# rust-bio/rust-bio

Measured on NVIDIA H100. Metric: GCUPS, higher is better.
Workload: dtype int32

## Files before the change

rust_bio_b200/csrc/b2a_common.cuh:

```cuda
#pragma once
#include <stdint.h>

#if defined(__CUDACC__)
#define B2A_HD __host__ __device__ __forceinline__
#else
#define B2A_HD inline
struct int4 { int x, y, z, w; };
struct int2 { int x, y; };
struct uint4 { unsigned x, y, z, w; };
inline int4 make_int4(int x, int y, int z, int w) { return int4{x, y, z, w}; }
inline int2 make_int2(int x, int y) { return int2{x, y}; }
#endif

namespace b2a {

#if defined(B2A_HOST_WARP) && !defined(__CUDACC__)
struct HostWarp {
  long long x[32];
  void (*next_lane)(void*);
  void* harness;
  void (*other_warp)(void*);
};
inline HostWarp* host_warp = nullptr;
inline int host_lane = 0;
// ... 51 lines not shown
  uint32_t uniform;
  uint32_t nstrips;
  uint32_t xwords;
  uint32_t ywords;
  uint32_t K;
  uint32_t rows_pad;
  uint64_t seq_off;
  uint64_t bnd_off;
  uint64_t rows_off;
  uint64_t rowm_off;
  uint64_t tb_off;
  uint64_t ops_off;
  uint64_t strip_task_base;
};

enum { ROWS_SN = 0, ROWS_LY = 1, ROWS_SL = 2, ROWS_IL = 3, ROWS_NL = 4, ROWS_ARRAYS = 5 };

B2A_HD int32_t imax(int32_t a, int32_t b) { return a > b ? a : b; }


B2A_HD int32_t col0_I(const DevScoring& sc, int32_t i) {
  if (i == 1) return sc.gap_open;
  return imax(sc.gap_open + sc.gap_extend * (i - 1), sc.xclip_prefix + sc.gap_open);
}
B2A_HD uint32_t col0_ibits(const DevScoring& sc, int32_t i) {
  if (i == 1) return TB_START;
  return (sc.gap_open + sc.gap_extend * (i - 1) > sc.xclip_prefix + sc.gap_open) ? TB_INS
                                                                                   : TB_XCLIP_PREFIX;
}
B2A_HD int32_t col0_S(const DevScoring& sc, int32_t i) {
  return imax(col0_I(sc, i), sc.xclip_prefix);
}
B2A_HD uint32_t col0_sbits(const DevScoring& sc, int32_t i) {
  return sc.xclip_prefix > col0_I(sc, i) ? TB_XCLIP_PREFIX : TB_INS;
}
B2A_HD int32_t row0_D(const DevScoring& sc, int32_t j) {
  if (j == 1) return sc.gap_open;
  return imax(sc.gap_open + sc.gap_extend * (j - 1), sc.yclip_prefix + sc.gap_open);
}
B2A_HD uint32_t row0_dbits(const DevScoring& sc, int32_t j) {
  if (j == 1) return TB_START;
  return (sc.gap_open + sc.gap_extend * (j - 1) > sc.yclip_prefix + sc.gap_open) ? TB_DEL
                                                                                   : TB_YCLIP_PREFIX;
}
B2A_HD int32_t row0_S(const DevScoring& sc, int32_t j, int32_t n) {
  int32_t s = imax(row0_D(sc, j), sc.yclip_prefix);
  if (j == n && sc.yclip_suffix > s) s = sc.yclip_suffix;
  return s;
}
B2A_HD uint32_t row0_sbits(const DevScoring& sc, int32_t j, int32_t n) {
  if (j == 0) return TB_START;
  const int32_t d = row0_D(sc, j);
  uint32_t b = d > sc.yclip_prefix ? TB_DEL : TB_YCLIP_PREFIX;
  if (j == n && sc.yclip_suffix > imax(d, sc.yclip_prefix)) b = TB_YCLIP_SUFFIX;
  return b;
}
B2A_HD int32_t xclip_score(const DevScoring& sc, int32_t j) {
  return sc.xclip_prefix + imax(sc.yclip_prefix, sc.gap_open + sc.gap_extend * (j - 1));
}

B2A_HD int64_t bnd_index(int32_t G, int32_t j, int32_t pi, int32_t maxn) {
  return G < 32 ? (int64_t)j * 32 + pi : (int64_t)pi * (maxn + 1) + j;
}

B2A_HD int32_t pack_s16x2(int32_t lo, int32_t hi) {
#if defined(__CUDA_ARCH__)
  return (int32_t)__byte_perm((uint32_t)lo, (uint32_t)hi, 0x5410);
#else
  return (int32_t)(((uint32_t)hi << 16) | ((uint32_t)lo & 0xffffu));
#endif
}
B2A_HD int32_t lo_s16(int32_t w) { return (int32_t)(int16_t)(uint16_t)((uint32_t)w & 0xffffu); }
B2A_HD int32_t hi_s16(int32_t w) { return w >> 16; }

#if defined(__CUDACC__)
__host__ __device__
#endif
constexpr int lut_entries(int alpha) { return (alpha + 1) * alpha; }
#if defined(__CUDACC__)
__host__ __device__
#endif
constexpr uint32_t lut_smem_bytes(int alpha) { return ((uint32_t)lut_entries(alpha) * 4u + 127u) & ~127u; }
constexpr int32_t LUT_POISON = 2;

#ifndef B2A_W_8_20
#define B2A_W_8_20 4
#endif
#if defined(__CUDACC__)
__host__ __device__
#endif
constexpr int fill_warps_of(int G, int R) { return (G == 8 && R == 20) ? B2A_W_8_20 : 4; }
#if defined(__CUDACC__)
__host__ __device__
#endif
constexpr bool cap_dispatch_of(int G) { return G == 8; }

#if defined(__CUDACC__)
__host__ __device__
#endif
constexpr int tbw_of(int R) { return (R + 3) / 4; }

}
```

rust_bio_b200/csrc/b2a_engine.cu:

```cuda
#include <cuda_runtime.h>

#include <chrono>
#include <cstdio>
#include <cstdlib>
#include <cstring>
#include <cub/device/device_scan.cuh>
#include <string>
#include <vector>

#define B2A_DEFINE_WALK_KERNEL
#include "../../include/b200align.h"
#include "b2a_fill_launch.h"
#include "b2a_kernels.cuh"
#include "b2a_plan.h"
#include "b2a_walk.cuh"
#include "b2a_banded.cuh"
#include "b2a_banded_strip.cuh"

using namespace b2a;

namespace {

struct DevBuf {
  void* p = nullptr;
// ... 610 lines not shown
      CK(cudaMallocHost(&e->h_plan, need + need / 4));
      e->h_plan_cap = need + need / 4;
    }
    size_t pos = 0;
    auto up_staged = [&](DevBuf& bf, const void* src, size_t bytes) -> cudaError_t {
      if (!bytes) return cudaSuccess;
      std::memcpy(e->h_plan + pos, src, bytes);
      const cudaError_t ce = up(bf, e->h_plan + pos, bytes);
      pos += (bytes + 15) & ~(size_t)15;
      return ce;
    };
    CK(up_staged(e->d_order, pl.order.data(), n * 4));
    CK(up_staged(e->d_pm, pl.pm.data(), n * 4));
    CK(up_staged(e->d_pn, pl.pn.data(), n * 4));
    CK(up_staged(e->d_blocks, pl.blocks.data(), blocks_bytes));
    CK(up_staged(e->d_codemap, e->codemap_host, 256));
    if (lut_b) CK(up_staged(e->d_lut, e->lut_host.data(), lut_b));
  }
  if (!e->stage_nosync) CK(cudaStreamSynchronize(st));
  e->score_only = score_only;
  e->staged = true;
  return B2A_OK;
}

int32_t b2a_batch_stage(b2a_engine* e, int32_t mode, const b2a_scoring* s, const b2a_pairs* pairs) {
  return batch_stage_impl(e, mode, s, pairs, false);
}

int32_t b2a_batch_stage_scores(b2a_engine* e, int32_t mode, const b2a_scoring* s, const b2a_pairs* pairs) {
  return batch_stage_impl(e, mode, s, pairs, true);
}

int32_t b2a_batch_run(b2a_engine* e) {
  if (!e) return B2A_E_INVALID;
  if (!e->staged) return e->fail(B2A_E_STATE, "b2a_batch_run before b2a_batch_stage");
  if (cudaSetDevice(e->device) != cudaSuccess) return e->fail(B2A_E_NO_DEVICE, "cudaSetDevice failed");
  const Plan& pl = e->plan;
  cudaStream_t st = e->stream;
  const FillLaunchFn fill = e->score_only ? e->shape->launch_notb : e->shape->launch;
  void (*const walk_warp_k)(const WalkParams) = e->score_only ? walk_warp_kernel<true> : walk_warp_kernel<false>;
  void (*const walk_lane_k)(const WalkParams) = e->score_only ? walk_kernel<true> : walk_kernel<false>;
  const bool use_tail = e->is_slot && e->tail_stream != nullptr && pl.waves.size() == 1;
  e->tail_used = use_tail;
  e->launches = 0;
  uint32_t* ctl = e->d_ctl.as<uint32_t>();
  CK(cudaMemsetAsync(ctl, 0, 256, st));
  CK(cudaEventRecord(e->ev[0], st));
  if (!pl.blocks.empty()) {
    PackParams pk{};
    pk.blocks = e->d_blocks.as<Block>();
    pk.order = e->d_order.as<uint32_t>();
    pk.blob = e->d_blob.as<uint8_t>();
    pk.x_off = e->d_xoff.as<uint64_t>();
    pk.x_len = e->d_xlen.as<uint32_t>();
    pk.y_off = e->d_yoff.as<uint64_t>();
    pk.y_len = e->d_ylen.as<uint32_t>();
    pk.codemap = e->d_codemap.as<uint8_t>();
    pk.seq = e->d_seq.as<uint8_t>();
    pk.bad_symbol = ctl;
    pk.G = pl.G;
    pack_kernel<<<(unsigned)pl.blocks.size(), 256, 0, st>>>(pk);
    CK(cudaGetLastError());
    ++e->launches;
  }
  CK(cudaEventRecord(e->ev[1], st));
  size_t wi = 0;
  for (const Wave& w : pl.waves) {
    const uint32_t nb = w.block_hi - w.block_lo;
    if (wi >= 60) return e->fail(B2A_E_UNSUPPORTED, "more than 60 traceback waves; raise the budget");
    FillParams fp{};
    fp.blocks = e->d_blocks.as<Block>() + w.block_lo;
    fp.nblocks = nb;
    fp.pm = e->d_pm.as<uint32_t>();
    fp.pn = e->d_pn.as<uint32_t>();
    fp.seq = e->d_seq.as<uint8_t>();
    fp.bnd = e->d_bnd.as<uint8_t>();
    fp.rows = e->d_rows.as<uint8_t>();
    fp.tb = e->score_only ? nullptr : e->d_tb.as<uint8_t>();
    fp.lut = e->d_lut.as<int32_t>() + (size_t)e->sc.alpha * e->sc.alpha;
    fp.task_counter = ctl + 2 + wi;
    fp.smem_seq_bytes = pl.smem_seq_bytes;
    fp.one = 1;
    fp.ge4 = 4 * e->sc.gap_extend;
    uint32_t fill_tasks = nb * (uint32_t)pl.G;
    if (pl.G == 32 && w.strip_tasks >= 0x7fffffffull) return e->fail(B2A_E_RANGE, "too many strip tasks in one wave");
    if (pl.G == 32 && w.strip_tasks > 0) {
      fp.progress = e->d_prog.as<uint32_t>();
      fp.n_strip_tasks = (uint32_t)w.strip_tasks;
      fill_tasks = fp.n_strip_tasks;
      CK(cudaMemsetAsync(fp.progress, 0, (size_t)w.strip_tasks * 4, st));
    }
    fp.sc = e->sc;
    while (e->wave_ev.size() < 3 * (wi + 1)) {
      cudaEvent_t v;
      CK(cudaEventCreate(&v));
      e->wave_ev.push_back(v);
    }
    WalkParams wp{};
    wp.blocks = fp.blocks;
    wp.nblocks = nb;
    wp.pm = fp.pm;
    wp.pn = fp.pn;
    wp.order = e->d_order.as<uint32_t>();
    wp.seq = fp.seq;
    wp.bnd = fp.bnd;
    wp.rows = fp.rows;
    wp.rowm = e->d_rowm.as<uint8_t>();
    wp.tb = fp.tb;
    wp.ops_scratch = e->d_opsscratch.as<uint8_t>();
    wp.lut = e->d_lut.as<int32_t>();
    wp.sc = e->sc;
    wp.G = pl.G;
    wp.R = pl.R;
    wp.packtrk = (e->flags & F_PACKTRK) ? 1 : 0;
    wp.bnd8 = (e->flags & F_BND8) ? 1 : 0;
    wp.filter_clips = (e->mode == B2A_MODE_SEMIGLOBAL || e->mode == B2A_MODE_LOCAL) ? 1 : 0;
    wp.score = e->d_score.as<int32_t>();
    wp.xstart = e->d_xs.as<uint32_t>();
    wp.xend = e->d_xe.as<uint32_t>();
    wp.ystart = e->d_ys.as<uint32_t>();
    wp.yend = e->d_ye.as<uint32_t>();
    wp.n_ops = e->d_nops.as<uint32_t>();
    wp.ops_src = e->d_opssrc.as<uint64_t>();
    wp.clip_len = e->d_clip.as<uint32_t>();
    wp.status = e->d_status.as<uint32_t>();
    wp.err_flag = ctl + 1;
    const bool fuse = false;
    fp.task_limit = (pl.G == 32) ? 0u : e->fill_task_limit;
    const uint64_t wave_pairs = (uint64_t)nb * 32;
    const bool warp_walk = e->walk_mode == 2 || (e->walk_mode == 0 && wave_pairs <= kWarpWalkMaxPairs);
    uint32_t per_warp_smem = 0;
    uint32_t wcta_warps = e->walk_cta_warps;
    if (warp_walk) {
      const uint32_t per_warp = ((pl.maxm + 3) / 4 + (pl.maxn + 3) / 4) * 4 + 16;
      if (!wcta_warps) wcta_warps = (uint64_t)per_warp * 8 <= 96 * 1024 ? 8u : 4u;
      per_warp_smem = (uint64_t)per_warp * wcta_warps <= 96 * 1024 ? per_warp : 0u;
      if ((size_t)per_warp_smem * wcta_warps > 48 * 1024)
        CK(cudaFuncSetAttribute(walk_warp_k, cudaFuncAttributeMaxDynamicSharedMemorySize, (int)(per_warp_smem * wcta_warps)));
    }
    if (!wcta_warps) wcta_warps = 4;
    wp.seq_smem_per_warp = per_warp_smem;
    const bool overlap_big = e->overlap_big && pl.waves.size() == 1 && !warp_walk && pl.G != 32 && nb >= 4096 && !use_tail;
    const bool overlap = overlap_big || (e->overlap_small && pl.waves.size() == 1 && warp_walk && pl.G != 32 && nb >= 64 &&
                                         !use_tail && e->walk_mode != 1);
    uint32_t split_b = 0;
    if (e->tail_split && !overlap && pl.waves.size() == 1 && warp_walk && pl.G != 32 && !use_tail && e->walk_mode != 1 &&
        fp.task_limit == 0) {
      int resident = 0;
      CK(fill(e->flags, fp, fill_tasks, e->num_sms, st, &resident, 1));
      const uint32_t slots = (uint32_t)resident, tasks = fill_tasks;
      if (slots > 0 && tasks > slots) {
        const uint32_t rounds = tasks / slots, rem = tasks % slots;
        const uint32_t a_blocks = (uint32_t)((uint64_t)rounds * slots / (uint32_t)pl.G);
        if (rem > 0 && rounds <= 6 && rem * 4 <= slots && a_blocks > 0 && a_blocks < nb) split_b = a_blocks;
      }
    }
    if (split_b) {
      if (!e->tail_stream) {
        int lo_pri = 0, hi_pri = 0;
        cudaDeviceGetStreamPriorityRange(&lo_pri, &hi_pri);
        CK(cudaStreamCreateWithPriority(&e->tail_stream, cudaStreamNonBlocking, hi_pri));
        CK(cudaEventCreateWithFlags(&e->ev_fill, cudaEventDisableTiming));
      }
      if (!e->aux_stream) CK(cudaStreamCreateWithFlags(&e->aux_stream, cudaStreamNonBlocking));
      while (e->sub_ev.size() < 6) {
        cudaEvent_t v;
// ... 1177 lines not shown
```

rust_bio_b200/csrc/b2a_fill.cuh:

```cuda
#pragma once
#include "b2a_common.cuh"

namespace b2a {

struct FillParams {
  const Block* blocks;
  uint32_t nblocks;
  const uint32_t* pm;
  const uint32_t* pn;
  const uint8_t* seq;
  uint8_t* bnd;
  uint8_t* rows;
  uint8_t* tb;
  const int32_t* lut;
  uint32_t* task_counter;
  uint32_t smem_seq_bytes;
  int32_t one;
  int32_t ge4;
  uint32_t* progress;
  uint32_t n_strip_tasks;
  uint32_t task_limit;
  DevScoring sc;
};

template <int G>
struct LaneCtx {
  DevScoring sc;
  const int32_t* lut;
  const uint32_t* xs;
  const uint32_t* ys;
  int32_t m, n;
  int32_t maxn;
  int32_t maxm;
  int32_t g;
  int32_t l;
  int32_t lane;
  int32_t pi;
  int32_t nstrips;
  int32_t K;
  int32_t rows_pad;
  bool uniform;
  int4* bnd;
  int32_t* rows;
  uint4* tb;
  uint32_t lut_base;
  uint32_t* prog_mine;
  uint32_t* prog_prev;
  int32_t only_strip;
  int32_t one;
  int32_t ge4;
};

#if defined(__CUDA_ARCH__)
#define B2A_SHFL_UP(v, G) __shfl_up_sync(0xffffffffu, (v), 1, (G))
#elif defined(B2A_HOST_WARP) && !defined(__CUDACC__)
inline int32_t host_shfl_up_group(int32_t v, int G) {
  if (!host_warp) return v;
  const int me = host_lane;
  return (int32_t)host_warp_exchange(v, [&](const long long* x) { return (me % G) ? x[me - 1] : x[me]; });
}
#define B2A_SHFL_UP(v, G) host_shfl_up_group((v), (G))
#define B2A_SPIN_YIELD() host_spin_yield()
#else
#define B2A_SHFL_UP(v, G) (v)
#endif
#ifndef B2A_SPIN_YIELD
#define B2A_SPIN_YIELD() ((void)0)
#endif

constexpr int32_t NEG4 = -(1 << 30);

B2A_HD int32_t max3(int32_t a, int32_t b, int32_t c) {
#if defined(__CUDA_ARCH__)
  return __vimax3_s32(a, b, c);
#else
  return imax(a, imax(b, c));
#endif
}
B2A_HD int32_t max3_relu(int32_t a, int32_t b, int32_t c) {
#if defined(__CUDA_ARCH__)
  return __vimax3_s32_relu(a, b, c);
#else
  return imax(imax(a, imax(b, c)), 0);
#endif
}
B2A_HD int32_t imin(int32_t a, int32_t b) { return a < b ? a : b; }
B2A_HD int32_t addmax(int32_t a, int32_t b, int32_t c) {
#if defined(__CUDA_ARCH__)
  return __viaddmax_s32(a, b, c);
#else
  return imax(a + b, c);
#endif
}
B2A_HD int32_t addmin(int32_t a, int32_t b, int32_t c) {
#if defined(__CUDA_ARCH__)
  return __viaddmin_s32(a, b, c);
#else
  return imin(a + b, c);
#endif
}
B2A_HD int32_t scale4(int32_t v) { return v <= DEAD_CLIP ? NEG4 : 4 * v; }

B2A_HD int32_t fmad(int32_t a, int32_t k, int32_t b) {
#if defined(__CUDA_ARCH__)
  int32_t d;
  asm("mad.lo.s32 %0, %1, %2, %3;" : "=r"(d) : "r"(a), "r"(k), "r"(b));
  return d;
#else
  return a * k + b;
#endif
}
B2A_HD int32_t lut_at(const void* host_base, uint32_t byte_addr) {
#if defined(__CUDA_ARCH__)
  int32_t v;
  asm("ld.shared.s32 %0, [%1];" : "=r"(v) : "r"(byte_addr));
  return v;
#else
  return *reinterpret_cast<const int32_t*>(reinterpret_cast<const char*>(host_base) + byte_addr);
#endif
}

B2A_HD uint32_t ld_progress(const uint32_t* p) {
#if defined(__CUDA_ARCH__)
  return *reinterpret_cast<const volatile uint32_t*>(p);
#else
  return *p;
#endif
}
template <class T>
B2A_HD T ld_boundary(const T* p, bool bypass_l1) {
#if defined(__CUDA_ARCH__)
  return bypass_l1 ? __ldcg(p) : *p;
#else
  (void)bypass_l1;
  return *p;
#endif
}
B2A_HD void fence_device() {
#if defined(__CUDA_ARCH__)
  __threadfence();
#endif
}

constexpr int32_t KEY_NONE = (int32_t)0x80000000;

template <int G, int R, int FLAGS, bool MASKED, bool LAST, int CAPQ>
B2A_HD void column_step(const LaneCtx<G>& c, const int32_t j, const int32_t tstep, const int32_t q, const int32_t rowbase,
                        const int32_t rv, int32_t (&Sp)[R], int32_t (&Dp)[R], int32_t (&SnR)[R],
                        int32_t (&LyR)[R], uint32_t (&tbacc)[R], const int32_t (&xc)[R],
                        int32_t sdiag, int32_t& sup, int32_t& iup, int32_t& Tv, int32_t& Ti,
                        int32_t& cap_s, int32_t& cap_i) {
  constexpr bool TR = (FLAGS & F_TRACK_ROWS) != 0;
  constexpr bool TC = (FLAGS & F_TRACK_COLS) != 0;
  constexpr bool CX = (FLAGS & F_CLIPX) != 0;
  constexpr bool LUT = (FLAGS & F_LUT) != 0;
  constexpr bool PR = (FLAGS & F_PACKREL) != 0;
  constexpr bool PK = (FLAGS & F_PACKTRK) != 0 || PR;
  constexpr bool RELU = (FLAGS & F_RELU) != 0;
  constexpr bool NOTB = (FLAGS & F_NOTB) != 0;
  constexpr bool TMASK = MASKED && !LUT;
  const int32_t go4i = 4 * c.sc.gap_open + 2, go4d = 4 * c.sc.gap_open + 1, ge4 = c.ge4;
  const int32_t ma4 = 4 * c.sc.match_score + 3 - go4d, mi4 = 4 * c.sc.mismatch_score + 3 - go4d;
  const int32_t x4 = CX ? scale4(xclip_score(c.sc, j)) : 0;
  const int32_t xs4 = scale4(c.sc.xclip_suffix), ys4 = scale4(c.sc.yclip_suffix);
  const int32_t cj = 4095 - (PR ? (tstep & KREL_MASK) : j);
  const int32_t one = c.one, k2 = one + one, k16 = k2 * 8, k1024 = k16 * 64;
  const int32_t q4 = q * 4;
  const uint32_t capbit = (MASKED && rv >= 1) ? 1u << (rv - 1) : 0u;
  int32_t Tl = KEY_NONE;
  int32_t key_even = KEY_NONE;
  int32_t sdo = fmad(sdiag, one, go4d);
  int32_t iop = fmad(sup, one, go4i);
  int32_t s4 = sup;
#pragma unroll
  for (int r = 0; r < R; ++r) {
    int32_t sub4;
    if (LUT) {
      sub4 = lut_at(c.lut, (uint32_t)fmad(q4, one, xc[r]));
    } else {
      sub4 = (xc[r] == q) ? ma4 : mi4;
    }
    const int32_t m4 = fmad(sdo, one, sub4);
    const int32_t i4 = addmax(iup, ge4, iop);
    const int32_t dop = Sp[r];
    const int32_t d4 = addmax(Dp[r], ge4, dop);
    int32_t sP;
    if (CX && RELU) {
      sP = max3_relu(m4, i4, d4);
    } else {
      sP = max3(m4, i4, d4);
      if (CX) sP = imax(sP, x4);
    }
    s4 = sP & ~3;
    const int32_t fi = addmin(i4, -iop, 4), fd = addmin(d4, -dop, 4);
    const int32_t nib = fmad(fd, k2, fi) + sP - s4;
    if (!NOTB) tbacc[r] = (uint32_t)(fmad((int32_t)tbacc[r], k16, fmad(fd, k2, fi)) + sP - s4);
    if (TC) {
      if (PK) {
        if (TMASK) {
          if (r < rv) Tl = imax(Tl, fmad(s4, k1024, 4095 - r));
        } else {
          const int32_t key = fmad(s4, k1024, 4095 - r);
          if (r & 1) Tl = max3(Tl, key_even, key);
          else key_even = key;
        }
      } else {
        const int32_t v = s4 + xs4;
        if ((!TMASK || r < rv) && v > Tv) {
          Tv = v;
          Ti = rowbase + 1 + r;
        }
      }
    }
    if (TR) {
      if (PK) {
        SnR[r] = imax(SnR[r], fmad(s4, k1024, cj));
      } else {
        const int32_t v = s4 + ys4;
        if (v > SnR[r]) {
          SnR[r] = v;
          LyR[r] = j;
        }
      }
    }
    if (LAST) {
      const int32_t slot = (rowbase + 1 + r) * 32 + c.pi;
      c.rows[ROWS_SL * c.rows_pad * 32 + slot] = s4 >> 2;
      c.rows[ROWS_IL * c.rows_pad * 32 + slot] = i4 >> 2;
      c.rows[ROWS_NL * c.rows_pad * 32 + slot] = nib;
    }
    if (MASKED && (CAPQ < 0 || (r >> 2) == CAPQ)) {
      if ((capbit >> r) & 1u) {
        cap_s = s4;
        cap_i = i4;
      }
    }
    sdo = dop;
    Sp[r] = fmad(s4, one, go4d);
    iop = fmad(s4, one, go4i);
    Dp[r] = d4;
    iup = i4;
  }
  sup = s4;
  if (TC && PK) {
    if (Tl != KEY_NONE) Tv = imax(Tv, Tl - ((PR ? c.l * R : rowbase) + 1));
  }
}

template <int G, int R, int FLAGS, bool MASKED, int CAPQ>
B2A_HD void run_strip(const LaneCtx<G>& c, const int32_t s) {
  constexpr bool TR = (FLAGS & F_TRACK_ROWS) != 0;
  constexpr bool TC = (FLAGS & F_TRACK_COLS) != 0;
  constexpr bool LUT = (FLAGS & F_LUT) != 0;
  constexpr bool PR = (FLAGS & F_PACKREL) != 0;
  constexpr bool PK = (FLAGS & F_PACKTRK) != 0 || PR;
  constexpr bool B8 = (FLAGS & F_BND8) != 0;
  constexpr bool NOTB = (FLAGS & F_NOTB) != 0;
  static_assert(!B8 || ((FLAGS & F_PACKTRK) != 0 && !PR), "F_BND8 needs the packed column tracker with absolute rows");
  constexpr int P = 32 / G;
  constexpr int TBW = tbw_of(R);
  int2* const bnd8 = reinterpret_cast<int2*>(c.bnd);
  const int32_t m = c.m, n = c.n;
  const int32_t rowbase = s * (G * R) + c.l * R;
  int32_t rv = m - 1 - rowbase;
  rv = rv < 0 ? 0 : (rv > R ? R : rv);
  const int32_t ys = c.sc.yclip_suffix;

  int32_t Sp[R], Dp[R], SnR[R], LyR[R], xc[R];
  uint32_t tbacc[R];
#pragma unroll
  for (int w = 0; w < R / 4; ++w) {
    const uint32_t xw = c.xs[(rowbase / 4 + w) * P + c.g];
#pragma unroll
    for (int b = 0; b < 4; ++b) {
      const int32_t sym = (int32_t)((xw >> (8 * b)) & 0xffu);
      xc[w * 4 + b] = LUT ? (int32_t)(c.lut_base + (uint32_t)(sym * c.sc.alpha * 4)) : sym;
      if (MASKED && LUT && w * 4 + b >= rv) xc[w * 4 + b] = (int32_t)(c.lut_base + (uint32_t)(c.sc.alpha * c.sc.alpha * 4));
    }
  }
#pragma unroll
  for (int r = 0; r < R; ++r) {
    const int32_t i = rowbase + 1 + r;
    const int32_t s0 = col0_S(c.sc, i);
    Sp[r] = 4 * s0 + (4 * c.sc.gap_open + 1);
    Dp[r] = NEG4;
    tbacc[r] = 0;
    LyR[r] = 0;
    if (TR) {
      if (PK) {
        SnR[r] = s0 * 4096 + 4095;
      } else {
        const int32_t v = s0 + ys;
        SnR[r] = (ys > DEAD_CLIP && v > MIN_SCORE) ? 4 * v : NEG4;
      }
    } else {
      SnR[r] = 0;
    }
  }
  int32_t sup_prev = rowbase == 0 ? 0 : 4 * col0_S(c.sc, rowbase);
  const int32_t t_none = PK ? KEY_NONE : NEG4;
  int32_t in_s = 0, in_i = NEG4, in_tv = t_none, in_ti = m;
  int32_t up_tv = NEG4, up_ti = m;
  const int32_t xs4_pr = scale4(c.sc.xclip_suffix);
  auto flush_rows = [&](const int32_t chunk, int32_t (&SnRr)[R]) {
#pragma unroll
    for (int r = 0; r < R; ++r) {
      const int32_t slot = (rowbase + 1 + r) * 32 + c.pi;
      if (SnRr[r] != KEY_NONE) {
        const int32_t sn = (SnRr[r] >> 12) + ys;
        const int32_t step = (chunk << KREL_BITS) + (4095 - (SnRr[r] & 4095));
        if (sn > c.rows[ROWS_SN * c.rows_pad * 32 + slot]) {
          c.rows[ROWS_SN * c.rows_pad * 32 + slot] = sn;
          c.rows[ROWS_LY * c.rows_pad * 32 + slot] = step - c.l + 1;
        }
      }
      SnRr[r] = KEY_NONE;
    }
  };
  int4 pre = make_int4(0, 0, 0, 0);
  int2 pre8 = make_int2(0, 0);
  const bool top_from_mem = (c.l == 0) && (s > 0);
  const bool top_from_row0 = (c.l == 0) && (s == 0);
  uint32_t avail = 0;
  const bool piped = c.prog_mine != nullptr;
  auto wait_col = [&](int32_t col) {
    if (piped && c.prog_prev && (int32_t)avail < col) {
      do {
        avail = ld_progress(c.prog_prev);
        B2A_SPIN_YIELD();
      } while ((int32_t)avail < col);
      fence_device();
    }
  };
  const bool top_valid = top_from_mem && rv >= 1;
  if (top_valid && n >= 1) {
    wait_col(1);
    if (B8) pre8 = ld_boundary(&bnd8[bnd_index(G, 1, c.pi, c.maxn)], piped);
    else pre = ld_boundary(&c.bnd[bnd_index(G, 1, c.pi, c.maxn)], piped);
  }
  const bool writer =
      MASKED ? (rv >= 1 && (c.l == G - 1 || rowbase + R >= m - 1)) : (c.l == G - 1);
  int32_t cap_s = 0, cap_i = 0;
  uint32_t yw = 0;
  uint4* tbs = NOTB ? nullptr : c.tb + (size_t)s * c.K * TBW * 32;
  const int32_t nsteps = c.K * 8;

  if (PR && TR) {
#pragma unroll
    for (int r = 0; r < R; ++r) {
      const int32_t slot = (rowbase + 1 + r) * 32 + c.pi;
      c.rows[ROWS_SN * c.rows_pad * 32 + slot] = col0_S(c.sc, rowbase + 1 + r) + ys;
      c.rows[ROWS_LY * c.rows_pad * 32 + slot] = 0;
      SnR[r] = KEY_NONE;
    }
  }
  for (int32_t t0 = 0; t0 < nsteps; t0 += (PR ? (1 << KREL_BITS) : nsteps)) {
  const int32_t t1 = PR ? ((t0 + (1 << KREL_BITS) < nsteps) ? t0 + (1 << KREL_BITS) : nsteps) : nsteps;
  for (int32_t t = t0; t < t1; ++t) {
    const int32_t j = t - c.l + 1;
    const bool active = (j >= 1) && (j <= n);
    if (active) {
      int32_t q;
      if (G == 1) {
        if ((t & 3) == 0) yw = c.ys[(t >> 2) * P + c.g];
        q = (int32_t)(yw & 0xffu);
        yw >>= 8;
      } else {
        const int32_t jb = j - 1;
        q = (int32_t)((c.ys[(jb >> 2) * P + c.g] >> (8 * (jb & 3))) & 0xffu);
      }
      if (top_from_row0) {
        in_s = 4 * row0_S(c.sc, j, n);
        in_i = NEG4;
        in_tv = t_none;
        in_ti = m;
        if (PR) {
          up_tv = NEG4;
          up_ti = m;
        }
      } else if (top_from_mem) {
        if (B8) {
          in_s = lo_s16(pre8.x);
          in_i = hi_s16(pre8.x);
          if (TC) in_tv = fmad(pre8.y, c.one, 0);
        } else {
          in_s = pre.x;
          in_i = pre.y;
        }
        if (TC && !B8) {
          if (PR) {
            up_tv = pre.z;
            up_ti = pre.w;
            in_tv = KEY_NONE;
          } else {
            in_tv = pre.z;
            in_ti = pre.w;
          }
        }
        if (j < n && top_valid) {
          wait_col(j + 1);
          if (B8) pre8 = ld_boundary(&bnd8[bnd_index(G, j + 1, c.pi, c.maxn)], piped);
          else pre = ld_boundary(&c.bnd[bnd_index(G, j + 1, c.pi, c.maxn)], piped);
        }
      }
      int32_t sup = in_s, iup = in_i, Tv = in_tv, Ti = in_ti;
      if (j == n) {
        column_step<G, R, FLAGS, MASKED, true, CAPQ>(c, j, t, q, rowbase, rv, Sp, Dp, SnR, LyR, tbacc, xc,
                                               sup_prev, sup, iup, Tv, Ti, cap_s, cap_i);
      } else {
        column_step<G, R, FLAGS, MASKED, false, CAPQ>(c, j, t, q, rowbase, rv, Sp, Dp, SnR, LyR, tbacc, xc,
                                                sup_prev, sup, iup, Tv, Ti, cap_s, cap_i);
      }
      sup_prev = in_s;
      if (writer) {
        if (B8) {
          const int32_t s4 = (MASKED && rv < R) ? cap_s : sup, i4 = (MASKED && rv < R) ? cap_i : iup;
          bnd8[bnd_index(G, j, c.pi, c.maxn)] = make_int2(pack_s16x2(s4, i4), TC ? Tv : t_none);
        } else {
          int4 o;
          o.x = (MASKED && rv < R) ? cap_s : sup;
          o.y = (MASKED && rv < R) ? cap_i : iup;
          o.z = TC ? Tv : t_none;
          o.w = TC ? Ti : m;
          if (PR) {
            o.z = NEG4;
            o.w = m;
            if (TC) {
              o.z = up_tv;
              o.w = up_ti;
              if (Tv != KEY_NONE) {
                const int32_t loc_v = ((Tv >> 12) << 2) + xs4_pr;
                if (loc_v > up_tv) {
                  o.z = loc_v;
                  o.w = s * (G * R) + (4095 - (Tv & 4095));
                }
              }
            }
          }
          c.bnd[bnd_index(G, j, c.pi, c.maxn)] = o;
        }
        if (piped && ((j & 15) == 0 || j == n)) {
          fence_device();
          *reinterpret_cast<volatile uint32_t*>(c.prog_mine) = (uint32_t)j;
          B2A_SPIN_YIELD();
        }
      }
      in_s = sup;
      in_i = iup;
      in_tv = Tv;
      in_ti = Ti;
    } else if (!NOTB) {
#pragma unroll
      for (int r = 0; r < R; ++r) tbacc[r] <<= 4;
    }
    if (G > 1) {
      in_s = B2A_SHFL_UP(in_s, G);
      in_i = B2A_SHFL_UP(in_i, G);
      if (TC) {
        in_tv = B2A_SHFL_UP(in_tv, G);
        if (!PK) in_ti = B2A_SHFL_UP(in_ti, G);
        if (PR) {
          up_tv = B2A_SHFL_UP(up_tv, G);
          up_ti = B2A_SHFL_UP(up_ti, G);
        }
      }
    }
    if (!NOTB && (t & 7) == 7) {
      uint4* dst = tbs + (size_t)(t >> 3) * TBW * 32 + c.lane;
#pragma unroll
      for (int qd = 0; qd < TBW; ++qd) {
        uint4 v;
        v.x = tbacc[qd * 4 + 0];
        v.y = (qd * 4 + 1 < R) ? tbacc[qd * 4 + 1] : 0u;
        v.z = (qd * 4 + 2 < R) ? tbacc[qd * 4 + 2] : 0u;
        v.w = (qd * 4 + 3 < R) ? tbacc[qd * 4 + 3] : 0u;
        dst[qd * 32] = v;
      }
    }
  }
  if (PR && TR) flush_rows(t0 >> KREL_BITS, SnR);
  }
  if (TR && !PR) {
#pragma unroll
    for (int r = 0; r < R; ++r) {
      const int32_t slot = (rowbase + 1 + r) * 32 + c.pi;
      int32_t sn, ly;
      if (PK) {
        sn = (SnR[r] >> 12) + ys;
        ly = 4095 - (SnR[r] & 4095);
      } else {
        sn = (SnR[r] <= NEG4 / 2) ? MIN_SCORE : (SnR[r] >> 2);
        ly = LyR[r];
      }
      c.rows[ROWS_SN * c.rows_pad * 32 + slot] = sn;
      c.rows[ROWS_LY * c.rows_pad * 32 + slot] = ly;
    }
  }
}

template <int G, int R, int FLAGS>
B2A_HD void fill_lane(const LaneCtx<G>& c) {
  const int32_t s_lo = c.only_strip >= 0 ? c.only_strip : 0;
  const int32_t s_hi = c.only_strip >= 0 ? c.only_strip + 1 : c.nstrips;
  for (int32_t s = s_lo; s < s_hi; ++s) {
    const bool full = c.uniform && ((s + 1) * (G * R) <= c.maxm - 1);
    if (full) {
      run_strip<G, R, FLAGS, false, -1>(c, s);
    } else if (cap_dispatch_of(G) && c.uniform) {
      const int32_t left = c.maxm - 1 - s * (G * R);
      const int32_t part = (left > 0 && left < G * R) ? left % R : 0;
      switch (part ? (part - 1) >> 2 : R / 4) {
        case 0: run_strip<G, R, FLAGS, true, 0>(c, s); break;
        case 1: run_strip<G, R, FLAGS, true, (1 <= R / 4 ? 1 : -1)>(c, s); break;
        case 2: run_strip<G, R, FLAGS, true, (2 <= R / 4 ? 2 : -1)>(c, s); break;
        case 3: run_strip<G, R, FLAGS, true, (3 <= R / 4 ? 3 : -1)>(c, s); break;
        case 4: run_strip<G, R, FLAGS, true, (4 <= R / 4 ? 4 : -1)>(c, s); break;
        case 5: run_strip<G, R, FLAGS, true, (5 <= R / 4 ? 5 : -1)>(c, s); break;
        default: run_strip<G, R, FLAGS, true, -1>(c, s); break;
      }
    } else {
      run_strip<G, R, FLAGS, true, -1>(c, s);
    }
  }
}

#if defined(__CUDACC__)

__device__ __forceinline__ uint32_t smem_u32(const void* p) {
  return (uint32_t)__cvta_generic_to_shared(p);
}
__device__ __forceinline__ void mbar_init(uint64_t* bar, uint32_t count) {
  asm volatile("mbarrier.init.shared::cta.b64 [%0], %1;" ::"r"(smem_u32(bar)), "r"(count));
}
__device__ __forceinline__ void mbar_expect_tx(uint64_t* bar, uint32_t bytes) {
  asm volatile("mbarrier.arrive.expect_tx.shared::cta.b64 _, [%0], %1;" ::"r"(smem_u32(bar)),
               "r"(bytes)
               : "memory");
}
__device__ __forceinline__ void tma_bulk_g2s(void* dst_smem, const void* src_gmem, uint32_t bytes,
                                             uint64_t* bar) {
  asm volatile(
      "cp.async.bulk.shared::cluster.global.mbarrier::complete_tx::bytes [%0], [%1], %2, [%3];" ::"r"(
          smem_u32(dst_smem)),
      "l"(src_gmem), "r"(bytes), "r"(smem_u32(bar))
      : "memory");
}
__device__ __forceinline__ bool mbar_try_wait(uint64_t* bar, uint32_t parity) {
  uint32_t done;
  asm volatile(
      "{\n\t.reg .pred p;\n\t"
      "mbarrier.try_wait.parity.shared::cta.b64 p, [%1], %2;\n\t"
      "selp.b32 %0, 1, 0, p;\n\t}"
      : "=r"(done)
      : "r"(smem_u32(bar)), "r"(parity)
      : "memory");
  return done != 0;
}

#ifndef B2A_MINB
#define B2A_MINB 1
#endif

template <int G, int R, int FLAGS>
__global__ void __launch_bounds__(fill_warps_of(G, R) * 32, B2A_MINB) fill_kernel(const FillParams prm) {
  extern __shared__ __align__(128) uint8_t smem[];
  constexpr int P = 32 / G;
  constexpr int FILL_WARPS = fill_warps_of(G, R);
  constexpr bool LUT = (FLAGS & F_LUT) != 0;
  constexpr int TBW = tbw_of(R);
  const int warp = threadIdx.x >> 5, lane = threadIdx.x & 31;
  uint64_t* bars = reinterpret_cast<uint64_t*>(smem);
  int32_t* lut_s = reinterpret_cast<int32_t*>(smem + 64);
  const uint32_t lut_bytes = LUT ? lut_smem_bytes(prm.sc.alpha) : 0u;
  uint8_t* stage = smem + 64 + lut_bytes + (size_t)warp * prm.smem_seq_bytes;
  uint64_t* bar = &bars[warp];
  if (threadIdx.x < FILL_WARPS) mbar_init(&bars[threadIdx.x], 1);
  if (LUT) {
    for (int k = threadIdx.x; k < lut_entries(prm.sc.alpha); k += blockDim.x) lut_s[k] = prm.lut[k];
  }
  asm volatile("fence.mbarrier_init.release.cluster;" ::: "memory");
  __syncthreads();

  const bool strip_tasks = (G == 32) && prm.progress != nullptr;
  const uint32_t ntasks = strip_tasks ? prm.n_strip_tasks : prm.nblocks * G;
  uint32_t parity = 0;

  for (uint32_t done = 0; prm.task_limit == 0 || done < prm.task_limit; ++done) {
    uint32_t task = 0;
    if (lane == 0) task = atomicAdd(prm.task_counter, 1u);
    task = __shfl_sync(0xffffffffu, task, 0);
    if (task >= ntasks) break;
    uint32_t b, sub;
    int32_t only_strip = -1;
    if (strip_tasks) {
      uint32_t lo = 0, hi = prm.nblocks;
      while (hi - lo > 1) {
        const uint32_t mid = (lo + hi) / 2;
        if (prm.blocks[mid].strip_task_base <= task) lo = mid;
        else hi = mid;
      }
      b = lo;
      const uint32_t rel = task - (uint32_t)prm.blocks[b].strip_task_base;
      const uint32_t ns = prm.blocks[b].nstrips;
      sub = rel / ns;
      only_strip = (int32_t)(rel % ns);
    } else {
      b = task / G;
      sub = task % G;
    }
    const Block blk = prm.blocks[b];
    if (strip_tasks && sub >= blk.npairs) continue;
    const uint32_t xbytes = blk.xwords * P * 4, ybytes = blk.ywords * P * 4;
    const uint32_t xoff = strip_tasks ? (uint32_t)only_strip * G * R : 0u;
    const uint32_t xstage = strip_tasks ? (uint32_t)(G * R) : xbytes;
    if (lane == 0) {
      asm volatile("fence.proxy.async.shared::cta;" ::: "memory");
      mbar_expect_tx(bar, xstage + ybytes);
      const uint8_t* src = prm.seq + blk.seq_off;
      tma_bulk_g2s(stage, src + (size_t)sub * xbytes + xoff, xstage, bar);
      tma_bulk_g2s(stage + xstage, src + (size_t)G * xbytes + (size_t)sub * ybytes, ybytes, bar);
    }
    LaneCtx<G> c;
    c.sc = prm.sc;
    c.lut = lut_s;
    c.lut_base = smem_u32(lut_s);
    c.one = prm.one;
    c.ge4 = prm.ge4;
    c.only_strip = only_strip;
    c.prog_mine = strip_tasks ? prm.progress + task : nullptr;
    c.prog_prev = (strip_tasks && only_strip > 0) ? prm.progress + task - 1 : nullptr;
    c.xs = reinterpret_cast<const uint32_t*>(stage) - xoff / 4;
    c.ys = reinterpret_cast<const uint32_t*>(stage + xstage);
    c.g = lane / G;
    c.l = lane % G;
    c.lane = lane;
    c.pi = (int32_t)(sub * P) + c.g;
    const bool valid = (uint32_t)c.pi < blk.npairs;
    c.m = valid ? (int32_t)prm.pm[blk.first + c.pi] : 0;
    c.n = valid ? (int32_t)prm.pn[blk.first + c.pi] : 0;
    c.maxn = (int32_t)blk.maxn;
    c.maxm = (int32_t)blk.maxm;
    c.nstrips = (int32_t)blk.nstrips;
    c.K = (int32_t)blk.K;
    c.rows_pad = (int32_t)blk.rows_pad;
    c.uniform = blk.uniform != 0;
    c.bnd = reinterpret_cast<int4*>(prm.bnd + blk.bnd_off);
    c.rows = reinterpret_cast<int32_t*>(prm.rows + blk.rows_off);
    c.tb = (FLAGS & F_NOTB) ? nullptr
                            : reinterpret_cast<uint4*>(prm.tb + blk.tb_off) + (size_t)sub * blk.nstrips * blk.K * TBW * 32;
    while (!mbar_try_wait(bar, parity)) {
    }
    parity ^= 1u;
    fill_lane<G, R, FLAGS>(c);
    __syncwarp();
  }
}

#endif

}
```

rust_bio_b200/csrc/b2a_fill_inst.cu:

```cuda
#include "b2a_fill_launch.h"

#ifndef B2A_G
#error "compile with -DB2A_G=... -DB2A_R=..."
#endif

#ifdef B2A_NOTB
#define B2A_LAUNCH_NAME launch_fill_notb_
#else
#define B2A_LAUNCH_NAME launch_fill_
#endif

namespace b2a {

namespace {

template <int FLAGS>
cudaError_t go(const FillParams& prm, uint32_t ntasks, int num_sms, cudaStream_t stream,
               int* grid_out, int dry) {
  auto kern = fill_kernel<B2A_G, B2A_R, FLAGS>;
  constexpr int FILL_WARPS = fill_warps_of(B2A_G, B2A_R);
  const uint32_t lut_bytes = (FLAGS & F_LUT) ? lut_smem_bytes(prm.sc.alpha) : 0u;
  const size_t smem = 64 + lut_bytes + (size_t)FILL_WARPS * prm.smem_seq_bytes;
  cudaError_t err =
      cudaFuncSetAttribute(kern, cudaFuncAttributeMaxDynamicSharedMemorySize, (int)smem);
  if (err != cudaSuccess) return err;
  int per_sm = 0;
  err = cudaOccupancyMaxActiveBlocksPerMultiprocessor(&per_sm, kern, FILL_WARPS * 32, smem);
  if (err != cudaSuccess) return err;
  if (per_sm < 1) return cudaErrorLaunchOutOfResources;
  if (dry) {
    if (grid_out) *grid_out = num_sms * per_sm * FILL_WARPS;
    return cudaSuccess;
  }
  const uint32_t want = (ntasks + FILL_WARPS - 1) / FILL_WARPS;
  uint32_t grid = (uint32_t)(num_sms * per_sm);
  if (grid > want) grid = want;
  if (prm.task_limit) grid = (want + prm.task_limit - 1) / prm.task_limit;
  if (grid < 1) grid = 1;
  if (grid_out) *grid_out = (int)grid;
  kern<<<grid, FILL_WARPS * 32, smem, stream>>>(prm);
  return cudaGetLastError();
}

}

#define B2A_CAT2(a, b, c) a##b##_##c
#define B2A_CAT(a, b, c) B2A_CAT2(a, b, c)

cudaError_t B2A_CAT(B2A_LAUNCH_NAME, B2A_G, B2A_R)(int flags, const FillParams& prm, uint32_t ntasks,
                                                   int num_sms, cudaStream_t stream, int* grid_out, int dry) {
  constexpr int ALL = F_TRACK_ROWS | F_TRACK_COLS | F_CLIPX;
#ifdef B2A_NOTB
  constexpr int NOTB = F_NOTB;
#else
  constexpr int NOTB = 0;
#endif
#define B2A_CASE(F) \
  case (NOTB | (F)): return go<(NOTB | (F))>(prm, ntasks, num_sms, stream, grid_out, dry);
  switch (flags) {
    B2A_CASE(0)
    B2A_CASE(F_TRACK_ROWS)
    B2A_CASE(F_TRACK_ROWS | F_PACKTRK)
    B2A_CASE(ALL)
    B2A_CASE(ALL | F_PACKTRK)
    B2A_CASE(ALL | F_RELU)
    B2A_CASE(ALL | F_PACKTRK | F_RELU)
    B2A_CASE(F_LUT)
    B2A_CASE(F_LUT | F_TRACK_ROWS)
    B2A_CASE(F_LUT | F_TRACK_ROWS | F_PACKTRK)
    B2A_CASE(F_LUT | ALL)
    B2A_CASE(F_LUT | ALL | F_PACKTRK)
    B2A_CASE(F_LUT | ALL | F_RELU)
    B2A_CASE(F_LUT | ALL | F_PACKTRK | F_RELU)
    B2A_CASE(F_TRACK_ROWS | F_PACKTRK | F_BND8)
    B2A_CASE(ALL | F_PACKTRK | F_BND8)
    B2A_CASE(ALL | F_PACKTRK | F_RELU | F_BND8)
    B2A_CASE(F_LUT | F_TRACK_ROWS | F_PACKTRK | F_BND8)
    B2A_CASE(F_LUT | ALL | F_PACKTRK | F_BND8)
    B2A_CASE(F_LUT | ALL | F_PACKTRK | F_RELU | F_BND8)
    B2A_CASE(F_TRACK_ROWS | F_PACKREL)
    B2A_CASE(ALL | F_PACKREL)
    B2A_CASE(ALL | F_PACKREL | F_RELU)
    B2A_CASE(F_LUT | F_TRACK_ROWS | F_PACKREL)
    B2A_CASE(F_LUT | ALL | F_PACKREL)
    B2A_CASE(F_LUT | ALL | F_PACKREL | F_RELU)
    default: return cudaErrorInvalidValue;
  }
}

}
```

Measured before the change: 791.0.

## Add per-strip shared-memory query profile and two-deep boundary prefetch for G=1

For full strips using the substitution LUT, each warp now builds a query profile in shared memory: substitution scores for every alphabet symbol against the strip's R rows. The inner column step then fetches them with vectorized 128-bit shared loads instead of R separate LUT gathers. The profile is enabled only when it fits in opt-in shared memory without reducing blocks per SM. Separately, the G=1 byte-boundary path prefetches boundary values two columns ahead by unrolling the column loop by two. The cost is extra shared memory, profile build time per strip, and more code paths and register pressure.

```diff
diff --git a/rust_bio_b200/csrc/b2a_common.cuh b/rust_bio_b200/csrc/b2a_common.cuh
--- a/rust_bio_b200/csrc/b2a_common.cuh
+++ b/rust_bio_b200/csrc/b2a_common.cuh
@@ -157,6 +157,14 @@
 #endif
 constexpr uint32_t lut_smem_bytes(int alpha) { return ((uint32_t)lut_entries(alpha) * 4u + 127u) & ~127u; }
 constexpr int32_t LUT_POISON = 2;
+#if defined(__CUDACC__)
+__host__ __device__
+#endif
+constexpr uint32_t qprof_warp_bytes(int R, int alpha) { return (uint32_t)alpha * (uint32_t)R * 128u; }
+#if defined(__CUDACC__)
+__host__ __device__
+#endif
+constexpr bool qprof_of(int flags) { return (flags & F_LUT) != 0 && (flags & F_PACKREL) == 0; }
 
 #ifndef B2A_W_8_20
 #define B2A_W_8_20 4
diff --git a/rust_bio_b200/csrc/b2a_engine.cu b/rust_bio_b200/csrc/b2a_engine.cu
--- a/rust_bio_b200/csrc/b2a_engine.cu
+++ b/rust_bio_b200/csrc/b2a_engine.cu
@@ -716,6 +716,7 @@
     fp.smem_seq_bytes = pl.smem_seq_bytes;
     fp.one = 1;
     fp.ge4 = 4 * e->sc.gap_extend;
+    fp.qprof = pl.maxm >= 1u + (uint32_t)(pl.G * pl.R) ? 1u : 0u;
     uint32_t fill_tasks = nb * (uint32_t)pl.G;
     if (pl.G == 32 && w.strip_tasks >= 0x7fffffffull) return e->fail(B2A_E_RANGE, "too many strip tasks in one wave");
     if (pl.G == 32 && w.strip_tasks > 0) {
diff --git a/rust_bio_b200/csrc/b2a_fill.cuh b/rust_bio_b200/csrc/b2a_fill.cuh
--- a/rust_bio_b200/csrc/b2a_fill.cuh
+++ b/rust_bio_b200/csrc/b2a_fill.cuh
@@ -20,6 +20,7 @@
   uint32_t* progress;
   uint32_t n_strip_tasks;
   uint32_t task_limit;
+  uint32_t qprof;
   DevScoring sc;
 };
 
@@ -49,6 +50,12 @@
   int32_t only_strip;
   int32_t one;
   int32_t ge4;
+#if defined(B2A_SIM_QPROF) && !defined(__CUDACC__)
+  int32_t* prof = sim_qprof_region();
+#else
+  int32_t* prof = nullptr;
+#endif
+  uint32_t prof_base = 0;
 };
 
 #if defined(__CUDA_ARCH__)
@@ -119,6 +126,23 @@
   return *reinterpret_cast<const int32_t*>(reinterpret_cast<const char*>(host_base) + byte_addr);
 #endif
 }
+B2A_HD int4 prof_ld(const int32_t* host_base, uint32_t byte_addr) {
+#if defined(__CUDA_ARCH__)
+  int4 v;
+  asm volatile("ld.shared.v4.s32 {%0, %1, %2, %3}, [%4];" : "=r"(v.x), "=r"(v.y), "=r"(v.z), "=r"(v.w) : "r"(byte_addr));
+  return v;
+#else
+  return *reinterpret_cast<const int4*>(reinterpret_cast<const char*>(host_base) + byte_addr);
+#endif
+}
+B2A_HD void prof_st(int32_t* host_base, uint32_t byte_addr, int4 v) {
+#if defined(__CUDA_ARCH__)
+  asm volatile("st.shared.v4.s32 [%0], {%1, %2, %3, %4};" ::"r"(byte_addr), "r"(v.x), "r"(v.y), "r"(v.z), "r"(v.w)
+               : "memory");
+#else
+  *reinterpret_cast<int4*>(reinterpret_cast<char*>(host_base) + byte_addr) = v;
+#endif
+}
 
 B2A_HD uint32_t ld_progress(const uint32_t* p) {
 #if defined(__CUDA_ARCH__)
@@ -144,7 +168,7 @@
 
 constexpr int32_t KEY_NONE = (int32_t)0x80000000;
 
-template <int G, int R, int FLAGS, bool MASKED, bool LAST, int CAPQ>
+template <int G, int R, int FLAGS, bool MASKED, bool LAST, int CAPQ, bool QP>
 B2A_HD void column_step(const LaneCtx<G>& c, const int32_t j, const int32_t tstep, const int32_t q, const int32_t rowbase,
                         const int32_t rv, int32_t (&Sp)[R], int32_t (&Dp)[R], int32_t (&SnR)[R],
                         int32_t (&LyR)[R], uint32_t (&tbacc)[R], const int32_t (&xc)[R],
@@ -172,10 +196,24 @@
   int32_t sdo = fmad(sdiag, one, go4d);
   int32_t iop = fmad(sup, one, go4i);
   int32_t s4 = sup;
+  int32_t subq[R];
+  if constexpr (QP) {
+    const uint32_t pa = c.prof_base + (uint32_t)c.lane * 16u + (uint32_t)q * (uint32_t)(R * 128);
+#pragma unroll
+    for (int k = 0; k < R / 4; ++k) {
+      const int4 v = prof_ld(c.prof, pa + (uint32_t)k * 512u);
+      subq[4 * k + 0] = v.x;
+      subq[4 * k + 1] = v.y;
+      subq[4 * k + 2] = v.z;
+      subq[4 * k + 3] = v.w;
+    }
+  }
 #pragma unroll
   for (int r = 0; r < R; ++r) {
     int32_t sub4;
-    if (LUT) {
+    if (QP) {
+      sub4 = subq[r];
+    } else if (LUT) {
       sub4 = lut_at(c.lut, (uint32_t)fmad(q4, one, xc[r]));
     } else {
       sub4 = (xc[r] == q) ? ma4 : mi4;
@@ -247,7 +285,7 @@
   }
 }
 
-template <int G, int R, int FLAGS, bool MASKED, int CAPQ>
+template <int G, int R, int FLAGS, bool MASKED, int CAPQ, bool QP = false>
 B2A_HD void run_strip(const LaneCtx<G>& c, const int32_t s) {
   constexpr bool TR = (FLAGS & F_TRACK_ROWS) != 0;
   constexpr bool TC = (FLAGS & F_TRACK_COLS) != 0;
@@ -278,6 +316,18 @@
       if (MASKED && LUT && w * 4 + b >= rv) xc[w * 4 + b] = (int32_t)(c.lut_base + (uint32_t)(c.sc.alpha * c.sc.alpha * 4));
     }
   }
+  if constexpr (QP) {
+    static_assert(LUT && !MASKED && R % 4 == 0, "the query profile is built for full strips from the LUT");
+    for (int32_t a = 0; a < c.sc.alpha; ++a) {
+#pragma unroll
+      for (int k = 0; k < R / 4; ++k) {
+        const uint32_t e = (uint32_t)a * 4u;
+        const int4 v = make_int4(lut_at(c.lut, (uint32_t)xc[4 * k + 0] + e), lut_at(c.lut, (uint32_t)xc[4 * k + 1] + e),
+                                 lut_at(c.lut, (uint32_t)xc[4 * k + 2] + e), lut_at(c.lut, (uint32_t)xc[4 * k + 3] + e));
+        prof_st(c.prof, c.prof_base + (uint32_t)c.lane * 16u + (uint32_t)a * (uint32_t)(R * 128) + (uint32_t)k * 512u, v);
+      }
+    }
+  }
 #pragma unroll
   for (int r = 0; r < R; ++r) {
     const int32_t i = rowbase + 1 + r;
@@ -318,7 +368,8 @@
     }
   };
   int4 pre = make_int4(0, 0, 0, 0);
-  int2 pre8 = make_int2(0, 0);
+  constexpr bool PF2 = B8 && G == 1;
+  int2 pre8a = make_int2(0, 0), pre8b = make_int2(0, 0);
   const bool top_from_mem = (c.l == 0) && (s > 0);
   const bool top_from_row0 = (c.l == 0) && (s == 0);
   uint32_t avail = 0;
@@ -335,8 +386,15 @@
   const bool top_valid = top_from_mem && rv >= 1;
   if (top_valid && n >= 1) {
     wait_col(1);
-    if (B8) pre8 = ld_boundary(&bnd8[bnd_index(G, 1, c.pi, c.maxn)], piped);
-    else pre = ld_boundary(&c.bnd[bnd_index(G, 1, c.pi, c.maxn)], piped);
+    if (B8) {
+      pre8a = ld_boundary(&bnd8[bnd_index(G, 1, c.pi, c.maxn)], piped);
+      if (PF2 && n >= 2) {
+        wait_col(2);
+        pre8b = ld_boundary(&bnd8[bnd_index(G, 2, c.pi, c.maxn)], piped);
+      }
+    } else {
+      pre = ld_boundary(&c.bnd[bnd_index(G, 1, c.pi, c.maxn)], piped);
+    }
   }
   const bool writer =
       MASKED ? (rv >= 1 && (c.l == G - 1 || rowbase + R >= m - 1)) : (c.l == G - 1);
@@ -356,7 +414,11 @@
   }
   for (int32_t t0 = 0; t0 < nsteps; t0 += (PR ? (1 << KREL_BITS) : nsteps)) {
   const int32_t t1 = PR ? ((t0 + (1 << KREL_BITS) < nsteps) ? t0 + (1 << KREL_BITS) : nsteps) : nsteps;
-  for (int32_t t = t0; t < t1; ++t) {
+  for (int32_t t2 = t0; t2 < t1; t2 += (PF2 ? 2 : 1)) {
+#pragma unroll
+  for (int u = 0; u < (PF2 ? 2 : 1); ++u) {
+    const int32_t t = t2 + u;
+    int2& pre8 = u ? pre8b : pre8a;
     const int32_t j = t - c.l + 1;
     const bool active = (j >= 1) && (j <= n);
     if (active) {
@@ -397,7 +459,12 @@
             in_ti = pre.w;
           }
         }
-        if (j < n && top_valid) {
+        if (PF2) {
+          if (j + 2 <= n && top_valid) {
+            wait_col(j + 2);
+            pre8 = ld_boundary(&bnd8[bnd_index(G, j + 2, c.pi, c.maxn)], piped);
+          }
+        } else if (j < n && top_valid) {
           wait_col(j + 1);
           if (B8) pre8 = ld_boundary(&bnd8[bnd_index(G, j + 1, c.pi, c.maxn)], piped);
           else pre = ld_boundary(&c.bnd[bnd_index(G, j + 1, c.pi, c.maxn)], piped);
@@ -405,11 +472,11 @@
       }
       int32_t sup = in_s, iup = in_i, Tv = in_tv, Ti = in_ti;
       if (j == n) {
-        column_step<G, R, FLAGS, MASKED, true, CAPQ>(c, j, t, q, rowbase, rv, Sp, Dp, SnR, LyR, tbacc, xc,
-                                               sup_prev, sup, iup, Tv, Ti, cap_s, cap_i);
+        column_step<G, R, FLAGS, MASKED, true, CAPQ, QP>(c, j, t, q, rowbase, rv, Sp, Dp, SnR, LyR, tbacc, xc,
+                                                   sup_prev, sup, iup, Tv, Ti, cap_s, cap_i);
       } else {
-        column_step<G, R, FLAGS, MASKED, false, CAPQ>(c, j, t, q, rowbase, rv, Sp, Dp, SnR, LyR, tbacc, xc,
-                                                sup_prev, sup, iup, Tv, Ti, cap_s, cap_i);
+        column_step<G, R, FLAGS, MASKED, false, CAPQ, QP>(c, j, t, q, rowbase, rv, Sp, Dp, SnR, LyR, tbacc, xc,
+                                                    sup_prev, sup, iup, Tv, Ti, cap_s, cap_i);
       }
       sup_prev = in_s;
       if (writer) {
@@ -478,6 +545,7 @@
       }
     }
   }
+  }
   if (PR && TR) flush_rows(t0 >> KREL_BITS, SnR);
   }
   if (TR && !PR) {
@@ -505,7 +573,12 @@
   for (int32_t s = s_lo; s < s_hi; ++s) {
     const bool full = c.uniform && ((s + 1) * (G * R) <= c.maxm - 1);
     if (full) {
-      run_strip<G, R, FLAGS, false, -1>(c, s);
+      if constexpr (qprof_of(FLAGS)) {
+        if (c.prof) run_strip<G, R, FLAGS, false, -1, true>(c, s);
+        else run_strip<G, R, FLAGS, false, -1>(c, s);
+      } else {
+        run_strip<G, R, FLAGS, false, -1>(c, s);
+      }
     } else if (cap_dispatch_of(G) && c.uniform) {
       const int32_t left = c.maxm - 1 - s * (G * R);
       const int32_t part = (left > 0 && left < G * R) ? left % R : 0;
@@ -572,7 +645,9 @@
   uint64_t* bars = reinterpret_cast<uint64_t*>(smem);
   int32_t* lut_s = reinterpret_cast<int32_t*>(smem + 64);
   const uint32_t lut_bytes = LUT ? lut_smem_bytes(prm.sc.alpha) : 0u;
-  uint8_t* stage = smem + 64 + lut_bytes + (size_t)warp * prm.smem_seq_bytes;
+  const uint32_t prof_bytes = (qprof_of(FLAGS) && prm.qprof) ? qprof_warp_bytes(R, prm.sc.alpha) : 0u;
+  uint8_t* prof = smem + 64 + lut_bytes + (size_t)warp * prof_bytes;
+  uint8_t* stage = smem + 64 + lut_bytes + (size_t)FILL_WARPS * prof_bytes + (size_t)warp * prm.smem_seq_bytes;
   uint64_t* bar = &bars[warp];
   if (threadIdx.x < FILL_WARPS) mbar_init(&bars[threadIdx.x], 1);
   if (LUT) {
@@ -626,6 +701,8 @@
     c.lut_base = smem_u32(lut_s);
     c.one = prm.one;
     c.ge4 = prm.ge4;
+    c.prof = prof_bytes ? reinterpret_cast<int32_t*>(prof) : nullptr;
+    c.prof_base = smem_u32(prof);
     c.only_strip = only_strip;
     c.prog_mine = strip_tasks ? prm.progress + task : nullptr;
     c.prog_prev = (strip_tasks && only_strip > 0) ? prm.progress + task - 1 : nullptr;
diff --git a/rust_bio_b200/csrc/b2a_fill_inst.cu b/rust_bio_b200/csrc/b2a_fill_inst.cu
--- a/rust_bio_b200/csrc/b2a_fill_inst.cu
+++ b/rust_bio_b200/csrc/b2a_fill_inst.cu
@@ -20,7 +20,7 @@
   auto kern = fill_kernel<B2A_G, B2A_R, FLAGS>;
   constexpr int FILL_WARPS = fill_warps_of(B2A_G, B2A_R);
   const uint32_t lut_bytes = (FLAGS & F_LUT) ? lut_smem_bytes(prm.sc.alpha) : 0u;
-  const size_t smem = 64 + lut_bytes + (size_t)FILL_WARPS * prm.smem_seq_bytes;
+  size_t smem = 64 + lut_bytes + (size_t)FILL_WARPS * prm.smem_seq_bytes;
   cudaError_t err =
       cudaFuncSetAttribute(kern, cudaFuncAttributeMaxDynamicSharedMemorySize, (int)smem);
   if (err != cudaSuccess) return err;
@@ -28,6 +28,24 @@
   err = cudaOccupancyMaxActiveBlocksPerMultiprocessor(&per_sm, kern, FILL_WARPS * 32, smem);
   if (err != cudaSuccess) return err;
   if (per_sm < 1) return cudaErrorLaunchOutOfResources;
+  FillParams p = prm;
+  p.qprof = 0;
+  if (qprof_of(FLAGS) && prm.qprof) {
+    const size_t smem_q = smem + (size_t)FILL_WARPS * qprof_warp_bytes(B2A_R, prm.sc.alpha);
+    int dev = 0, optin = 0, per_sm_q = 0;
+    err = cudaGetDevice(&dev);
+    if (err == cudaSuccess) err = cudaDeviceGetAttribute(&optin, cudaDevAttrMaxSharedMemoryPerBlockOptin, dev);
+    if (err != cudaSuccess) return err;
+    if (smem_q <= (size_t)optin) {
+      err = cudaFuncSetAttribute(kern, cudaFuncAttributeMaxDynamicSharedMemorySize, (int)smem_q);
+      if (err == cudaSuccess) err = cudaOccupancyMaxActiveBlocksPerMultiprocessor(&per_sm_q, kern, FILL_WARPS * 32, smem_q);
+      if (err != cudaSuccess) return err;
+      if (per_sm_q == per_sm) {
+        smem = smem_q;
+        p.qprof = 1;
+      }
+    }
+  }
   if (dry) {
     if (grid_out) *grid_out = num_sms * per_sm * FILL_WARPS;
     return cudaSuccess;
@@ -38,7 +56,7 @@
   if (prm.task_limit) grid = (want + prm.task_limit - 1) / prm.task_limit;
   if (grid < 1) grid = 1;
   if (grid_out) *grid_out = (int)grid;
-  kern<<<grid, FILL_WARPS * 32, smem, stream>>>(prm);
+  kern<<<grid, FILL_WARPS * 32, smem, stream>>>(p);
   return cudaGetLastError();
 }
 
```

After: 801.0 (median of 6 runs). +1.3%, better.
